# ywz978020607/MASIC

Measured on AMD Instinct MI355X. Metric: stereo pairs/sec (enc+dec), higher is better.
Workload: dtype bf16; 1 GPU; HSIC(N=128,M=192,K=5) eval forward (enc+dec both views), 8x3x512x512 stereo pairs per GPU (BASELINE.json configs[1] shape), inputs resident in HBM (the graph's static input buffers); the device homography of batch k+1 is handed over with batch k (one-batch look-ahead of a loader): its device->host read, the float32 host chain and the upload of the sampling matrices are done every step, under the r; pairs_per_gpu=8, height=512, width=512, parallelism=dp1 (pairs sharded, no data-path collective)

## Files before the change

coremasic/mywork/MASIC.py:

```python
import math
import os

import numpy as np

import torch
import torch.nn as nn
import torch.nn.functional as F

from compressai.entropy_models import (EntropyBottleneck, GaussianConditional, GaussianMixtureConditional,
                                       GaussianMixtureConditional_gf)
from compressai.layers import GDN, MaskedConv2d, ResidualBlock, conv3x3
from compressai.models.utils import conv, deconv, update_registered_buffers
from masic_amd import ops as _hip
from masic_amd.homography import warp_matrices as _warp_matrices
from masic_amd import autograd as _ag
from masic_amd.streams import ForkJoin as _ForkJoin
from masic_amd import fp8 as _fp8
from masic_amd import deconv as _deconv
from masic_amd import conv_s2 as _conv_s2
from masic_amd import latent as _latent
from masic_amd.bands import check_band_rows as _check_band_rows
from masic_amd.f16k import F16K as _F16K, F8K as _F8K

_RELU, _LEAKY, _NONE = _hip.ACT_RELU, _hip.ACT_LEAKY, _hip.ACT_NONE
_CAT_F16K = True
_HEADS_GROUPED = True


class CompressionModel(nn.Module):

    def __init__(self, entropy_bottleneck_channels, init_weights=True):
        super().__init__()
        self.entropy_bottleneck1 = EntropyBottleneck(entropy_bottleneck_channels)
        self.entropy_bottleneck2 = EntropyBottleneck(entropy_bottleneck_channels)
        if init_weights:
            self._initialize_weights()

    def aux_loss(self):
        return sum(m.loss() for m in self.modules() if isinstance(m, EntropyBottleneck))

    def _initialize_weights(self):
        for m in self.modules():
            if isinstance(m, (nn.Conv2d, nn.ConvTranspose2d)):
                nn.init.kaiming_normal_(m.weight)
                if m.bias is not None:
                    nn.init.zeros_(m.bias)

    def forward(self, *args):
        raise NotImplementedError()

    def parameters(self):
        for child in self.children():
            if not isinstance(child, EntropyBottleneck):
                yield from child.parameters()

    def aux_parameters(self):
        for child in self.children():
            if isinstance(child, EntropyBottleneck):
                yield from child.parameters()

    def update(self, force=False):
        for child in self.children():
            if isinstance(child, EntropyBottleneck):
                child.update(force=force)


class RateDistortionLoss(nn.Module):

    def __init__(self, lmbda=1e-2):
        super().__init__()
        self.lmbda = lmbda

    def forward(self, output, target):
        N, _, H, W = target.size()
        n = N * H * W
        bpp = sum(_hip.sum_log(l.contiguous()) for l in output["likelihoods"].values()) / (-math.log(2) * n)
        mse = _hip.sse(output["x_hat"].contiguous(), target.contiguous()) / target.numel()
        return {"bpp_loss": bpp.float(), "mse_loss": mse.float(), "loss": (self.lmbda * 255 ** 2 * mse + bpp).float()}


class AverageMeter:
    def __init__(self):
        self.val = self.avg = self.sum = self.count = 0

    def update(self, val, n=1):
        self.val = val
        self.sum += val * n
        self.count += n
        self.avg = self.sum / self.count


_SIDE_STREAMS = {}


def _side_streams(device, n=4):
    key = torch.device(device).index
    pool = _SIDE_STREAMS.get(key)
    if pool is None:
        pool, seen = [], set()
        for _ in range(64):
            s = torch.cuda.Stream(device=device)
            if s.cuda_stream not in seen:
                seen.add(s.cuda_stream)
                pool.append(s)
            if len(pool) == n + 1:
                break
        pool = _SIDE_STREAMS[key] = tuple(pool)
    cur = torch.cuda.current_stream(device).cuda_stream
    return tuple(s for s in pool if s.cuda_stream != cur)[:n]


_TRAIN_STREAMS = os.environ.get("MASIC_TRAIN_STREAMS", "1") != "0"


def _keep_until(t, stream):
    if not (torch.is_tensor(t) or isinstance(t, _F16K)):
        return
    if not torch.cuda.is_current_stream_capturing():
        t.record_stream(stream)


def _bf16_inference(*tensors):
    from masic_amd import nn as _mnn
    if not _mnn.reduced_precision():
        return False
    return not (torch.is_grad_enabled() and any(t.requires_grad for t in tensors))


def _f16k_chain(convs, acts, x, in_op=0, out=None, out_coff=0, gate=None, gate_c=0):
    B, _, H, W = x.shape
    hw = (H, W)
    for cv in convs:
        if not cv.f16k_supported(B, *hw):
            return None
        hw = cv.out_hw(*hw)
    t = x if isinstance(x, _F16K) else _F16K.from_nchw(x, in_op=in_op)
    for cv, act in zip(convs[:-1], acts):
        t = cv.run_f16k(t, act=act)
    return convs[-1].run_f16k(t, act=acts[-1], want_nchw=out is None, out=out, out_coff=out_coff, gate=gate, gate_c=gate_c)


def _pair_conv(conv, xa, xb, gdn_in=None, gdn_out=None):
    B, _, H, W = xa.shape
    desc = conv._desc((B, 6, H, W))
    def g(m):
        return None if m is None else (m.beta.detach(), m.gamma.detach().contiguous(), m.inverse)
    bm = (gdn_in or gdn_out).beta_min if (gdn_in or gdn_out) is not None else 1e-6
    return _hip.conv5s1_pair(xa, xb, conv.packed_weight(desc), None if conv.bias is None else conv.bias.detach(),
                             gdn_in=g(gdn_in), gdn_out=g(gdn_out), beta_min=bm)


def _gdn_f16k(gdn, x):
    return _hip.gdn_f16k(x, gdn.beta.detach(), gdn.gamma.detach(), inverse=gdn.inverse, beta_min=gdn.beta_min)


def _own_kernel_or_f16k(kernel, cv, gdn, t):
    if t.whole and kernel.supported(cv, gdn, t.B, t.H, t.W):
        return kernel.run(cv, gdn, t)
    return cv.run_f16k(t, gdn=gdn)


def _analysis_f16k(owner, x, layouts=None):
    from masic_amd import nn as _mnn
    convs = (owner.g_a_conv1, owner.g_a_conv2, owner.g_a_conv3, owner.g_a_conv4)
    gdns = (owner.g_a_gdn1, owner.g_a_gdn2, owner.g_a_gdn3)
    B, C, H, W = x.shape
    c1 = convs[0]
    if (C, c1.out_channels, tuple(c1.kernel_size), tuple(c1.stride), tuple(c1.padding)) != (3, 128, (5, 5), (2, 2), (2, 2)):
        return None
    sizes = [((H - 1) // 2 + 1, (W - 1) // 2 + 1)]
    for cv in convs[1:]:
        if not cv.f16k_supported(B, *sizes[-1]):
            return None
# ... 87 lines not shown
                L = dict(x=t[k], bias=layer.bias.detach(), Cin=layer.in_channels, Cout=layer.out_channels, act=acts[i],
                         out="nchw" if i == 2 else "f16k")
                if sc is not None and i < 2:
                    L["wp"], L["ws"] = layer.packed_gemm_f8k_weight(sc["c"] if i == 0 else sc[tag])
                    if i == 0:
                        L["out"], L["out_scale"] = "f8k", sc[tag]
                else:
                    L["wp"] = layer.packed_gemm_dma_weight()
                layers.append(L)
            t = _hip.gemm_f16k_group(layers, B, H, W)
        return tuple(t)

    def _f8k_heads_ok(self):
        return all(seq[i].in_channels % 32 == 0 and seq[i].out_channels % 32 == 0 for seq in (self.gmm_sigma, self.gmm_means, self.gmm_weights) for i in (0, 2)) \
            and all(seq[4].in_channels % 16 == 0 and seq[4].out_channels % 32 == 0 for seq in (self.gmm_sigma, self.gmm_means, self.gmm_weights))

    def heads(self, x, parallel=True):
        from masic_amd import nn as _mnn
        if isinstance(x, _F16K):
            if not x.whole:
                raise RuntimeError(f"_GmmHeads.heads: the grouped GEMMs read a whole buffer, not {x!r}")
            return self._heads_grouped(x, None)
        if _mnn.reduced_precision() and not (torch.is_grad_enabled() and (x.requires_grad or self.gmm_sigma[0].weight.requires_grad)):
            B, _, H, W = x.shape
            sc = _fp8.scales(self)
            use_f8 = sc is not None and self._f8k_heads_ok()
            if use_f8:
                xv = _F8K(_hip.nchw_to_f8k(x, sc["c"]), *x.shape, sc["c"])
                branch = lambda seq, tag, acts: self._branch_f8k(seq, xv, sc, tag, acts)
            else:
                xv = _F16K.from_nchw(x)
                xf = xv.buf

                def branch(seq, tag, acts):
                    if _fp8.recording():
                        _fp8.record(self, "c", x)
                        l0 = seq[0]
                        _fp8.record(self, tag, _hip.gemm_f16k(xf, l0.packed_gemm_dma_weight(), l0.bias.detach(), B, l0.in_channels, l0.out_channels, H, W, acts[0])
                                    if l0.in_channels % 16 == 0 and l0.out_channels % 32 == 0 else
                                    _hip.gemm1x1_bf16(xf, l0.packed_gemm_weight(), l0.bias.detach(), B, l0.in_channels, l0.out_channels, H, W, acts[0]))
                    return self._branch_f16k(seq, xv, acts)
            if _HEADS_GROUPED and not _fp8.recording() and self._grouped_heads_ok():
                return self._heads_grouped(xv, sc if use_f8 else None)
            if not parallel:
                return (branch(self.gmm_sigma, "h_sigma", (_RELU, _RELU, _RELU)),
                        branch(self.gmm_means, "h_means", (_LEAKY, _LEAKY, _NONE)),
                        branch(self.gmm_weights, "h_weights", (_LEAKY, _LEAKY, _NONE)))
            fj = _ForkJoin()
            cur = fj.main
            side = _side_streams(x.device)[2:4]
            outs = [None, None, None]
            for i, (st, (seq, tag, acts)) in enumerate(zip(side, ((self.gmm_means, "h_means", (_LEAKY, _LEAKY, _NONE)),
                                                                  (self.gmm_weights, "h_weights", (_LEAKY, _LEAKY, _NONE))))):
                fj.fork(st)
                with fj.on(st):
                    outs[i + 1] = branch(seq, tag, acts)
            outs[0] = branch(self.gmm_sigma, "h_sigma", (_RELU, _RELU, _RELU))
            for st in side:
                fj.join(st)
            for t in outs[1:] + [xv.buf]:
                _keep_until(t, cur)
            return tuple(outs)
        if torch.is_grad_enabled() and _ag.gmm_heads_supported(self, x):
            return _ag.gmm_heads(self, x)
        sigma = self._branch(self.gmm_sigma, x, (_RELU, _RELU, _RELU))
        means = self._branch(self.gmm_means, x, (_LEAKY, _LEAKY, _NONE))
        logits = self._branch(self.gmm_weights, x, (_LEAKY, _LEAKY, _NONE))
        return sigma, means, logits

    def forward(self, x):
        sigma, means, logits = self.heads(x)
        return sigma, means, _hip.softmax_k(logits, self.K)


class gmm_hyper_y1_same_resolution(_GmmHeads):

    def __init__(self, N, M, K):
        super().__init__()
        self.N, self.M, self.K = N, M, K
        self.gmm_sigma = nn.Sequential(
            deconv(4 * M, 6 * M, kernel_size=1, stride=1), nn.ReLU(inplace=True),
            deconv(6 * M, 4 * M, kernel_size=1, stride=1), nn.ReLU(inplace=True),
            conv(4 * M, M * K, kernel_size=1, stride=1), nn.ReLU(inplace=True))
        self.gmm_means = nn.Sequential(
            deconv(4 * M, 6 * M, kernel_size=1, stride=1), nn.LeakyReLU(inplace=True),
            deconv(6 * M, 4 * M, kernel_size=1, stride=1), nn.LeakyReLU(inplace=True),
            conv(4 * M, M * K, kernel_size=1, stride=1))
        self.gmm_weights = nn.Sequential(
            deconv(4 * M, 6 * M, kernel_size=1, stride=1), nn.LeakyReLU(inplace=True),
            deconv(6 * M, M * K, kernel_size=1, stride=1), nn.LeakyReLU(inplace=True),
            conv(M * K, M * K, kernel_size=1, stride=1))


class gmm_hyper_y2_same_resolution(_GmmHeads):

    def __init__(self, N, M, K):
        super().__init__()
        self.N, self.M, self.K = N, M, K
        self.gmm_sigma = nn.Sequential(
            conv(5 * M, 6 * M, kernel_size=1, stride=1), nn.ReLU(inplace=True),
            conv(6 * M, 4 * M, kernel_size=1, stride=1), nn.ReLU(inplace=True),
            conv(4 * M, M * K, kernel_size=1, stride=1), nn.ReLU(inplace=True))
        self.gmm_means = nn.Sequential(
            conv(5 * M, 6 * M, kernel_size=1, stride=1), nn.LeakyReLU(inplace=True),
            conv(6 * M, 4 * M, kernel_size=1, stride=1), nn.LeakyReLU(inplace=True),
            conv(4 * M, M * K, kernel_size=1, stride=1))
        self.gmm_weights = nn.Sequential(
            conv(5 * M, 6 * M, kernel_size=1, stride=1), nn.LeakyReLU(inplace=True),
            conv(6 * M, M * K, kernel_size=1, stride=1), nn.LeakyReLU(inplace=True),
            conv(M * K, M * K, kernel_size=1, stride=1))


class mask2weights(nn.Module):

    def __init__(self, N, M, Kw):
        super().__init__()
        self.maskconv = nn.Sequential(
            conv(1, 3, kernel_size=3, stride=2), nn.ReLU(inplace=True),
            conv(3, 6, kernel_size=3), nn.ReLU(inplace=True),
            conv(6, 6, kernel_size=3), nn.ReLU(inplace=True),
            conv(6, 3, kernel_size=3))
        self.N, self.M, self.Kw = N, M, Kw

    def forward(self, m):
        s = self.maskconv
        t = s[0].run(m, act=_RELU)
        t = s[2].run(t, act=_RELU)
        t = s[4].run(t, act=_RELU)
        return s[6].run(t, act=_hip.ACT_SOFTMAX_C)


def _synthesis_f16k(dec, y_hat):
    B, _, H, W = y_hat.shape
    convs = (dec.g_s_conv1, dec.g_s_conv2, dec.g_s_conv3)
    gdns = (dec.g_s_gdn1, dec.g_s_gdn2, dec.g_s_gdn3)
    sizes = [(H, W)]
    for cv in convs:
        if cv.out_channels != 128 or not cv.f16k_supported(B, *sizes[-1]):
            return None
        sizes.append(cv.out_hw(*sizes[-1]))
    if not dec.g_s_conv4.d2s_supported(B, *sizes[3]):
        return None
    t = y_hat if isinstance(y_hat, _F16K) else _F16K.from_nchw(y_hat)
    sc = _fp8.scales(dec)
    if sc is not None and convs[1].f8k_supported(B, *sizes[1]) and convs[2].f8k_supported(B, *sizes[2]):
        t = convs[0].run_f16k_f8out(t, sc["d1"], gdn=gdns[0])
        t = convs[1].run_f8k(t, gdn=gdns[1], out="f8k", out_scale=sc["d2"])
        t = convs[2].run_f8k(t, gdn=gdns[2], out="f16k")
        return dec.g_s_conv4.run_f16k_d2s(t)
    for i in range(3):
        t = _own_kernel_or_f16k(_deconv, convs[i], gdns[i], t)
        if i < 2:
            _fp8.record(dec, "d%d" % (i + 1), t.buf)
    return dec.g_s_conv4.run_f16k_d2s(t)


class Encoder1(nn.Module):

    def __init__(self, N, M, **kwargs):
        super().__init__()
        self.g_a_conv1 = conv(3, N)
        self.g_a_gdn1 = GDN(N)
        self.g_a_conv2 = conv(N, N)
        self.g_a_gdn2 = GDN(N)
        self.g_a_conv3 = conv(N, N)
        self.g_a_gdn3 = GDN(N)
        self.g_a_conv4 = conv(N, M)

    def forward(self, x):
        g1 = self.g_a_gdn1(self.g_a_conv1(x))
        g2 = self.g_a_gdn2(self.g_a_conv2(g1))
        g3 = self.g_a_gdn3(self.g_a_conv3(g2))
        return self.g_a_conv4(g3), g1, g2, g3

    def latent(self, x):
        if _bf16_inference(x, self.g_a_conv1.weight):
            y = _analysis_f16k(self, x.contiguous())
            if y is not None:
                return y
        return self.forward(x)[0]

    def latent_layouts(self, x, **layouts):
        if _bf16_inference(x, self.g_a_conv1.weight):
            return _analysis_f16k(self, x.contiguous(), layouts=layouts)
        return None

    def latent_train(self, x):
        if _ag.analysis_supported(self, x):
            return _ag.analysis(self, x)
        return self.forward(x)[0]


class Decoder1(nn.Module):

    def __init__(self, N, M, **kwargs):
        super().__init__()
        self.g_s_conv1 = deconv(M, N)
        self.g_s_gdn1 = GDN(N, inverse=True)
        self.g_s_conv2 = deconv(N, N)
        self.g_s_gdn2 = GDN(N, inverse=True)
        self.g_s_conv3 = deconv(N, N)
        self.g_s_gdn3 = GDN(N, inverse=True)
        self.g_s_conv4 = deconv(N, 3)

    def forward(self, y_hat):
        g1 = self.g_s_gdn1(self.g_s_conv1(y_hat))
        g2 = self.g_s_gdn2(self.g_s_conv2(g1))
        g3 = self.g_s_gdn3(self.g_s_conv3(g2))
        return self.g_s_conv4(g3), g1, g2, g3

    def reconstruct(self, y_hat):
        if isinstance(y_hat, _F16K):
            return _synthesis_f16k(self, y_hat) if _bf16_inference(self.g_s_conv1.weight) else None
        if _bf16_inference(y_hat, self.g_s_conv1.weight):
            x_hat = _synthesis_f16k(self, y_hat)
            if x_hat is not None:
                return x_hat
        return self.forward(y_hat)[0]

    def reconstruct_train(self, y_hat):
        if _ag.synthesis_supported(self, y_hat):
            return _ag.synthesis(self, y_hat)
        return self.forward(y_hat)[0]


class Encoder2(nn.Module):

    def __init__(self, N, M, **kwargs):
        super().__init__()
        self.pre_conv = conv(6, 3, stride=1)
        self.pre_gdn = GDN(3)
        self.g_a_conv1 = conv(3, N)
        self.g_a_gdn1 = GDN(N)
        self.g_a_conv2 = conv(N, N)
        self.g_a_gdn2 = GDN(N)
        self.g_a_conv3 = conv(N, N)
        self.g_a_gdn3 = GDN(N)
        self.g_a_conv4 = conv(N, M)

    def forward(self, x1_warp, x2):
        if not (torch.is_grad_enabled() and (x1_warp.requires_grad or x2.requires_grad or self.pre_conv.weight.requires_grad)):
            return self.forward_views(x1_warp, x2)
        return self.forward_pair(_ag.cat(x1_warp, x2))

    def forward_views(self, x1_warp, x2, layouts=None):
        t = _pair_conv(self.pre_conv, x1_warp.contiguous(), x2.contiguous(), gdn_out=self.pre_gdn)
        if layouts is not None and _bf16_inference(t, self.g_a_conv1.weight):
            lay = _analysis_f16k(self, t, layouts=layouts)
            if lay is not None:
                return lay
        return self._analysis(t)

    def forward_pair(self, pair):
        return self._analysis(self.pre_gdn(self.pre_conv(pair)))

    def _analysis(self, t):
        if _bf16_inference(t, self.g_a_conv1.weight):
            y = _analysis_f16k(self, t)
            if y is not None:
                return y
        if torch.is_grad_enabled() and _ag.analysis_supported(self, t):
            return _ag.analysis(self, t)
        t = self.g_a_gdn1(self.g_a_conv1(t))
        t = self.g_a_gdn2(self.g_a_conv2(t))
        t = self.g_a_gdn3(self.g_a_conv3(t))
        return self.g_a_conv4(t)


class Decoder2(nn.Module):

    def __init__(self, N, M, **kwargs):
        super().__init__()
        self.g_s_conv1 = deconv(M, N)
        self.g_s_gdn1 = GDN(N, inverse=True)
        self.g_s_conv2 = deconv(N, N)
        self.g_s_gdn2 = GDN(N, inverse=True)
        self.g_s_conv3 = deconv(N, N)
        self.g_s_gdn3 = GDN(N, inverse=True)
        self.g_s_conv4 = deconv(N, 3)
        self.after_gdn = GDN(3, inverse=True)
        self.after_conv = deconv(6, 3, stride=1)

    def forward(self, y_hat, x1_hat_warp):
        if isinstance(y_hat, _F16K):
            t = _synthesis_f16k(self, y_hat) if _bf16_inference(x1_hat_warp, self.g_s_conv1.weight) else None
            if t is None:
                return None
        else:
            t = _synthesis_f16k(self, y_hat) if _bf16_inference(y_hat, self.g_s_conv1.weight) else None
        if t is None and torch.is_grad_enabled() and _ag.synthesis_supported(self, y_hat):
            t = _ag.synthesis(self, y_hat)
        if t is None:
            t = self.g_s_gdn1(self.g_s_conv1(y_hat))
            t = self.g_s_gdn2(self.g_s_conv2(t))
            t = self.g_s_gdn3(self.g_s_conv3(t))
            t = self.g_s_conv4(t)
        if not (torch.is_grad_enabled() and (t.requires_grad or x1_hat_warp.requires_grad or self.after_conv.weight.requires_grad)):
            return _pair_conv(self.after_conv, t.contiguous(), x1_hat_warp.contiguous(), gdn_in=self.after_gdn)
        t = self.after_gdn(t)
        return self.after_conv(_ag.cat(t, x1_hat_warp))


def mask(im1, H_inv):
    B, _, h, w = im1.shape
    m_fwd, m_back = _warp_matrices(H_inv, (h, w), (h, w), want_inverse=True)
    mask_r = _hip.warp_perspective(None, m_fwd, (h, w), ones_like=(B, h, w))
# ... 967 lines not shown
```

masic_amd/nn.py:

```python
import torch
import torch.nn as nn

import os

from . import ops
from .f16k import F16K, F8K
from ._lib import PREC_BF16, PREC_F32, PREC_FP8

_PRECISION = {"f32": PREC_F32, "bf16": PREC_BF16, "fp8": PREC_BF16}[os.environ.get("MASIC_PRECISION", "f32")]
_FP8 = os.environ.get("MASIC_PRECISION", "f32") == "fp8"


def set_precision(name):
    global _PRECISION, _FP8
    _PRECISION = {"f32": PREC_F32, "bf16": PREC_BF16, "fp8": PREC_BF16}[name]
    _FP8 = name == "fp8"


def get_precision():
    return "fp8" if _FP8 else ("bf16" if _PRECISION == PREC_BF16 else "f32")


def reduced_precision():
    return _PRECISION == PREC_BF16
# ... 31 lines not shown
        for k, v in m.__dict__.items():
            if k.endswith("_cache") and isinstance(v, tuple):
                stack = list(v[1:])
                while stack:
                    x = stack.pop()
                    if isinstance(x, torch.Tensor):
                        out.append(x)
                    elif isinstance(x, dict):
                        stack.extend(x.values())
                    elif isinstance(x, (tuple, list)):
                        stack.extend(x)
    return out


def packed_gdn_f16k(gdn):
    key = weight_key(gdn.beta) + weight_key(gdn.gamma)
    cache = gdn.__dict__.get("_packed_f16k_cache")
    if cache is None or cache[0] != key:
        cache = (key, ops.pack_gdn_f16k(gdn.beta.detach(), gdn.gamma.detach().contiguous(), gdn.beta_min))
        gdn.__dict__["_packed_f16k_cache"] = cache
    return cache[1]


class _PackedWeightMixin:
    transposed_conv = False
    masked_conv = False

    def _geometry(self):
        kh, kw = _pair(self.kernel_size)
        sh, sw = _pair(self.stride)
        ph, pw = _pair(self.padding)
        if sh != sw or ph != pw or _pair(self.dilation) != (1, 1) or self.groups != 1:
            raise RuntimeError("masic_amd: only square stride/padding, dilation 1, groups 1 convolutions are built")
        if self.transposed_conv and _pair(self.output_padding) != (sh - 1, sh - 1):
            raise RuntimeError("masic_amd: ConvTranspose2d needs output_padding = stride - 1 (compressai deconv())")
        return kh, kw, sh, ph

    def _desc(self, x_shape, in_ctot=None, in_coff=0, out_ctot=None, out_coff=0, in_op=ops.INOP_NONE,
              act=ops.ACT_NONE, gate_ctot=0, gate_c=0):
        kh, kw, s, p = self._geometry()
        B, _, Hi, Wi = x_shape
        return ops.make_conv_desc(B, self.in_channels, Hi, Wi, self.out_channels, kh, kw, s, p,
                                  transposed=self.transposed_conv, masked=self.masked_conv,
                                  in_ctot=in_ctot, in_coff=in_coff, out_ctot=out_ctot, out_coff=out_coff,
                                  in_op=in_op, act=act, gate_ctot=gate_ctot, gate_c=gate_c, prec=_PRECISION)

    def packed_weight(self, desc):
        w = self.weight
        return _cached(self, "_packed_cache", weight_key(w), (desc.B, desc.Hi, desc.Wi, desc.prec),
                       lambda: ops.pack_conv_weight(w.detach().contiguous(), desc))

    def packed_gemm_weight(self):
        w = self.weight
        key = weight_key(w)
        cache = self.__dict__.get("_packed_gemm_cache")
        if cache is None or cache[0] != key:
            cache = (key, ops.pack_gemm1x1_weight(w.detach().contiguous(), self.in_channels, self.out_channels, self.transposed_conv))
            self.__dict__["_packed_gemm_cache"] = cache
        return cache[1]

    def out_hw(self, Hi, Wi):
        kh, kw, s, p = self._geometry()
        return ops.conv_out_hw(Hi, Wi, kh, kw, s, p, self.transposed_conv)

    def _desc_f16k(self, B, Hi, Wi, out_ctot=None, out_coff=0, act=ops.ACT_NONE, gate_ctot=0, gate_c=0, in_ctot=None, in_coff=0):
        kh, kw, s, p = self._geometry()
        cin16 = (self.in_channels + 15) // 16 * 16
        return ops.make_conv_desc(B, self.in_channels, Hi, Wi, self.out_channels, kh, kw, s, p,
                                  transposed=self.transposed_conv, masked=self.masked_conv,
                                  in_ctot=cin16 if in_ctot is None else in_ctot, in_coff=in_coff,
                                  out_ctot=out_ctot, out_coff=out_coff, act=act, gate_ctot=gate_ctot, gate_c=gate_c, prec=PREC_BF16)

    def _desc_of(self, x, out=None, out_coff=0, act=ops.ACT_NONE, gate=None, gate_c=0, blk=16, nchw=False):
        if x.C != self.in_channels:
            raise RuntimeError(f"masic_amd: a layer of {self.in_channels} input channels on {x!r}")
        if isinstance(out, F16K):
            out_ctot, out_coff = out.ctot, out.coff
            if (out.B, out.C, out.H, out.W) != (x.B, self.out_channels) + self.out_hw(x.H, x.W):
                raise RuntimeError(f"masic_amd: {out!r} is not the output of this layer on {x!r}")
        elif out is not None:
            out_ctot = out.shape[1]
        else:
            out_ctot = None if nchw else (self.out_channels + blk - 1) // blk * blk
        return self._desc_f16k(x.B, x.H, x.W, out_ctot=out_ctot, out_coff=out_coff, act=act, gate_ctot=0 if gate is None else gate.shape[1],
                               gate_c=gate_c if gate is not None else 0, in_ctot=x.ctot, in_coff=x.coff)

    def _f16k_out(self, buf, desc, out=None):
        return out if out is not None else F16K(buf, desc.B, self.out_channels, desc.Ho, desc.Wo, desc.out_ctot, 0)

    def f16k_supported(self, B, Hi, Wi):
        return ops.conv_f16k_supported(self._desc_f16k(B, Hi, Wi))

    def packed_f16k_weight(self, desc):
        w = self.weight
        return _cached(self, "_packed_f16k_cache", weight_key(w), (desc.B, desc.Hi, desc.Wi),
                       lambda: ops.pack_conv_f16k_weight(w.detach().contiguous(), desc, persistent=w.is_contiguous() and not self.masked_conv))

    def _bias(self):
        return None if self.bias is None else self.bias.detach()

    def _desc_f8k(self, B, Hi, Wi, out_ctot=None, out_coff=0, act=ops.ACT_NONE, gate_ctot=0, gate_c=0):
        kh, kw, s, p = self._geometry()
        cin32 = (self.in_channels + 31) // 32 * 32
        return ops.make_conv_desc(B, self.in_channels, Hi, Wi, self.out_channels, kh, kw, s, p,
                                  transposed=self.transposed_conv, masked=self.masked_conv, in_ctot=cin32,
                                  out_ctot=out_ctot, out_coff=out_coff, act=act, gate_ctot=gate_ctot, gate_c=gate_c, prec=PREC_FP8)

    def f8k_supported(self, B, Hi, Wi):
        return self.in_channels % 32 == 0 and ops.conv_f16k_supported(self._desc_f8k(B, Hi, Wi))

    def run_f8k(self, x, act=ops.ACT_NONE, out="f16k", out_scale=None, out_nchw=None, out_coff=0, gate=None, gate_c=0, gdn=None):
        B, Hi, Wi = x.B, x.H, x.W
        gct = 0 if gate is None else gate.shape[1]
        if out_nchw is not None:
            desc = self._desc_f8k(B, Hi, Wi, out_ctot=out_nchw.shape[1], out_coff=out_coff, act=act, gate_ctot=gct, gate_c=gate_c)
        elif out == "nchw":
            desc = self._desc_f8k(B, Hi, Wi, act=act)
        else:
            blk = 32 if out == "f8k" else 16
            desc = self._desc_f8k(B, Hi, Wi, out_ctot=(self.out_channels + blk - 1) // blk * blk, act=act)
        w = self.weight
        vkey = weight_key(w)
        wp, ws = _cached(self, "_packed_f8k_cache", vkey, (desc.B, desc.Hi, desc.Wi), lambda: ops.pack_conv_f8k_weight(w.detach().contiguous(), desc))
        wscale = _cached(self, "_wscale_f8k_cache", vkey, (desc.B, desc.Hi, desc.Wi, float(x.scale)), lambda: (ws * float(x.scale)).contiguous())
        y = ops.conv2d_f8k(x.buf, wp, wscale, self._bias(), desc, out=out, out_scale=out_scale, out_nchw=out_nchw,
                           gate=gate, gdn=None if gdn is None else (packed_gdn_f16k(gdn), gdn.inverse))
        if out_nchw is not None or out == "nchw":
            return y
        if out == "f8k":
            return F8K(y, B, self.out_channels, desc.Ho, desc.Wo, out_scale)
        return self._f16k_out(y, desc)

    def run_f16k_f8out(self, x, out_scale, act=ops.ACT_NONE, gdn=None):
        desc = self._desc_of(x, act=act, blk=32)
        y = ops.conv2d_f8k(x.buf, self.packed_f16k_weight(desc), None, self._bias(), desc, out="f8k",
                           out_scale=out_scale, gdn=None if gdn is None else (packed_gdn_f16k(gdn), gdn.inverse))
        return F8K(y, x.B, self.out_channels, desc.Ho, desc.Wo, out_scale)

    def packed_gemm_f8k_weight(self, in_scale):
        w = self.weight
        vkey = weight_key(w)
        wp, ws = _cached(self, "_packed_gemm_f8k_cache", vkey, (), lambda: ops.pack_gemm_f8k_weight(w.detach().contiguous(), self.in_channels, self.out_channels, self.transposed_conv))
        return wp, _cached(self, "_wscale_gemm_f8k_cache", vkey, (float(in_scale),), lambda: (ws * float(in_scale)).contiguous())

    def packed_first_layer_weight(self):
        w = self.weight
        key = weight_key(w)
        cache = self.__dict__.get("_packed_conv_a_cache")
        if cache is None or cache[0] != key:
            cache = (key, ops.pack_conv_a_weight(w.detach().contiguous()))
            self.__dict__["_packed_conv_a_cache"] = cache
        return cache[1]

    def run_f16k_d2s(self, x, out=None, out_coff=0):
        if not self.transposed_conv or self._geometry() != (5, 5, 2, 2):
            raise RuntimeError("masic_amd: run_f16k_d2s is for ConvTranspose2d(k=5, s=2, p=2)")
        if not x.whole or x.C != self.in_channels:
            raise RuntimeError(f"masic_amd: run_f16k_d2s takes a whole tensor of {self.in_channels} channels, not {x!r}")
        B, Hi, Wi = x.B, x.H, x.W
        desc = ops.make_conv_desc(B, self.in_channels, Hi, Wi, 32, 3, 3, 1, 1, prec=PREC_BF16)
        w = self.weight

        def build():
            wc, bc = ops.deconv_s2_as_conv_weight_dev(w.detach().contiguous(), self._bias())
            return ops.pack_conv_f16k_weight(wc, desc), bc
        wp, bc = _cached(self, "_packed_d2s_cache", weight_key(w) + (None if self.bias is None else weight_key(self.bias),),
                         (B, Hi, Wi), build)
        return ops.conv2d_f16k_d2s(x.buf, wp, bc, desc, self.out_channels, out=out, out_coff=out_coff)

    def d2s_supported(self, B, Hi, Wi):
        return (self.transposed_conv and self._geometry() == (5, 5, 2, 2) and self.out_channels <= 8 and self.in_channels % 32 == 0
                and ops.conv_f16k_supported(ops.make_conv_desc(B, self.in_channels, Hi, Wi, 32, 3, 3, 1, 1, prec=PREC_BF16)))

    def run_f16k(self, x, act=ops.ACT_NONE, want_nchw=False, out=None, out_coff=0, gate=None, gate_c=0, gdn=None):
        to16 = isinstance(out, F16K)
        nchw = want_nchw or (out is not None and not to16)
        desc = self._desc_of(x, out, out_coff, act, gate if out is not None else None, gate_c, nchw=nchw)
        y = ops.conv2d_f16k(x.buf, self.packed_f16k_weight(desc), self._bias(), desc, out_nchw=None if to16 else out, want_nchw=want_nchw, gate=gate,
                            gdn=None if gdn is None else (packed_gdn_f16k(gdn), gdn.inverse), out16=out.buf if to16 else None)
        return y if nchw else self._f16k_out(y, desc, out)

    def f16k_multi_supported(self, B, Hi, Wi):
        return ops.conv_f16k_multi_supported(self._desc_f16k(B, Hi, Wi))

    def run_f16k_multi(self, x, want, round16=None, gate=None, gate_c=0):
        desc = self._desc_of(x, nchw=True)
        r = (None, 0, 0) if round16 is None else (round16.buf, round16.ctot, round16.coff)
        if round16 is not None and round16.shape != (x.B, self.out_channels, desc.Ho, desc.Wo):
            raise RuntimeError(f"masic_amd: {round16!r} is not the output of this layer on {x!r}")
        lay = ops.conv2d_f16k_multi(x.buf, self.packed_f16k_weight(desc), self._bias(), desc, want=want, round16=r[0], round16_ctot=r[1],
                                    round16_coff=r[2], gate=gate, gate_c=gate_c)
        for k in ("round16", "abs16"):
            if k in lay:
                lay[k] = round16 if (k == "round16" and round16 is not None) else F16K.wrap(lay[k], x.B, self.out_channels, desc.Ho, desc.Wo)
        return lay

    def run_f16k_dual(self, x, gdn, products=None):
        desc = self._desc_of(x)
        pre, y = ops.conv2d_f16k_gdn_dual(x.buf, self.packed_f16k_weight(desc), self._bias(), desc,
                                          (packed_gdn_f16k(gdn), gdn.inverse), products=products)
        return self._f16k_out(pre, desc), self._f16k_out(y, desc)

    def run_f16k_res(self, x, act=ops.ACT_NONE, res1=None, res2=None, out=None, y_pre=None):
        side = [r for r in (res1, res2, y_pre) if r is not None]
        res_ctot = side[0].ctot if side else 0
        for r in side:
            if not r.whole or r.ctot != res_ctot:
                raise RuntimeError(f"masic_amd: residual / pre-activation operands are whole tensors of one width, not {r!r}")
        res1, res2, y_pre = (None if r is None else r.buf for r in (res1, res2, y_pre))
        B, Hi, Wi = x.B, x.H, x.W
        if self.resident_supported(B, Hi, Wi) and act in (ops.ACT_NONE, ops.ACT_RELU, ops.ACT_LEAKY):
            w = self.weight
            wp = _cached(self, "_packed_c3_cache", weight_key(w), (), lambda: ops.pack_conv3x3_resident_weight(w.detach()))
            oc, ocoff = ((self.out_channels + 15) // 16 * 16, 0) if out is None else (out.ctot, out.coff)
            if not x.whole or (out is not None and out.shape != (B, self.out_channels, Hi, Wi)):
                raise RuntimeError(f"masic_amd: the resident-weight kernel takes a whole input and writes its own output, not {x!r} -> {out!r}")
            y = ops.conv3x3_resident(x.buf, wp, self._bias(), B, self.in_channels, self.out_channels, Hi, Wi, act=act, y16=None if out is None else out.buf,
                                     out_ctot=oc, out_coff=ocoff, res1=res1, res2=res2, res_ctot=res_ctot, y_pre=y_pre)
            return out if out is not None else F16K(y, B, self.out_channels, Hi, Wi, oc, 0)
        desc = self._desc_of(x, out, act=act)
        y = ops.conv2d_f16k_res(x.buf, self.packed_f16k_weight(desc), self._bias(), desc, y16=None if out is None else out.buf,
                                res1=res1, res2=res2, res_ctot=res_ctot, y_pre=y_pre)
        return self._f16k_out(y, desc, out)

    def resident_supported(self, B, Hi, Wi):
        return (not self.transposed_conv and not self.masked_conv and self._geometry() == (3, 3, 1, 1)
                and ops.conv3x3_resident_supported(B, self.in_channels, self.out_channels, Hi, Wi))

    def few_supported(self, B, Hi, Wi):
        kh, kw, s_, p_ = self._geometry()
        return (not self.transposed_conv and self.out_channels <= 32 and self.in_channels % 16 == 0
                and ops.conv_f16k_supported(ops.make_conv_desc(B, self.in_channels, Hi, Wi, 32, kh, kw, s_, p_, prec=PREC_BF16)))

    def run_f16k_few(self, x, res32=None):
        if not x.whole or x.C != self.in_channels:
            raise RuntimeError(f"masic_amd: run_f16k_few takes a whole tensor of {self.in_channels} channels, not {x!r}")
        B, Hi, Wi = x.B, x.H, x.W
        kh, kw, s_, p_ = self._geometry()
        desc = ops.make_conv_desc(B, self.in_channels, Hi, Wi, 32, kh, kw, s_, p_, prec=PREC_BF16)
        w = self.weight
        vkey = weight_key(w) + (None if self.bias is None else weight_key(self.bias),)

        def build():
            wpad = torch.zeros((32,) + tuple(w.shape[1:]), dtype=torch.float32, device=w.device)
            wpad[:self.out_channels] = w.detach()
            bpad = torch.zeros(32, dtype=torch.float32, device=w.device)
            if self.bias is not None:
                bpad[:self.out_channels] = self.bias.detach()
            return ops.pack_conv_f16k_weight(wpad, desc), bpad
        wp, bp = _cached(self, "_packed_few_cache", vkey, (B, Hi, Wi), build)
        return ops.conv2d_f16k_few(x.buf, wp, bp, desc, self.out_channels, res32=res32)

    def packed_gemm_dma_weight(self):
        w = self.weight
        key = weight_key(w)
        cache = self.__dict__.get("_packed_gemm_dma_cache")
        if cache is None or cache[0] != key:
            cache = (key, ops.pack_gemm_f16k_weight(w.detach().contiguous(), self.in_channels, self.out_channels, self.transposed_conv))
            self.__dict__["_packed_gemm_dma_cache"] = cache
        return cache[1]

    def run(self, x, in_coff=0, out=None, out_coff=0, in_op=ops.INOP_NONE, act=ops.ACT_NONE, gate=None, gate_c=0,
            res1=None, res2=None):
        if torch.is_grad_enabled() and (x.requires_grad or self.weight.requires_grad):
            return self._run_autograd(x, in_coff, out, in_op, act, gate, gate_c, res1, res2)
        desc = self._desc(x.shape, in_ctot=x.shape[1], in_coff=in_coff,
                          out_ctot=None if out is None else out.shape[1], out_coff=out_coff,
                          in_op=in_op, act=act, gate_ctot=0 if gate is None else gate.shape[1], gate_c=gate_c)
        bias = None if self.bias is None else self.bias.detach()
        return ops.conv2d(x, self.packed_weight(desc), bias, desc, out=out, gate=gate, res1=res1, res2=res2)

    def f16k_out_supported(self, shape):
        return reduced_precision() and ops.conv2d_f16k_out_supported(self._desc(tuple(shape), out_ctot=(self.out_channels + 15) // 16 * 16))

    def run_f16k_out(self, x, act=ops.ACT_NONE):
        desc = self._desc(tuple(x.shape), out_ctot=(self.out_channels + 15) // 16 * 16, act=act)
        return self._f16k_out(ops.conv2d_f16k_out(x, self.packed_weight(desc), self._bias(), desc), desc)

    def _run_autograd(self, x, in_coff, out, in_op, act, gate, gate_c, res1, res2):
        from . import autograd as A
        if out is not None:
            raise RuntimeError("masic_amd: writing into a concat buffer is an inference-only fusion; use autograd.CatFn when training")
        if in_coff != 0 or x.shape[1] != self.in_channels:
            raise RuntimeError("masic_amd: channel-slice inputs are an inference-only fusion")
        if in_op == ops.INOP_ABS:
            x = A.AbsFn.apply(x)
        elif in_op != ops.INOP_NONE:
            raise RuntimeError("masic_amd: round() inputs have no gradient path (eval-mode fusion)")
        if act == ops.ACT_SOFTMAX_C:
            y = A.SoftmaxKFn.apply(A.conv(self, x), self.out_channels)
        else:
            y = A.conv(self, x, act)
        if gate is not None:
            y = A.GateFn.apply(y, gate, gate_c)
        for r in (res1, res2):
            if r is not None:
                y = A.AddFn.apply(y, r)
        return y

    def forward(self, x):
        return self.run(x)


class Conv2d(_PackedWeightMixin, nn.Conv2d):
    pass


class ConvTranspose2d(_PackedWeightMixin, nn.ConvTranspose2d):
    transposed_conv = True

    def forward(self, x, output_size=None):
        if output_size is not None:
            raise RuntimeError("masic_amd: ConvTranspose2d(output_size=...) is not supported")
        return self.run(x)
```

Measured before the change: 4568 stereo pairs/s.

## Add warp-specialized persistent kernel for final depth-to-space deconv layer

Adds a dedicated HIP kernel for the last 128->C 5x5 stride-2 transposed conv, computed as a 3x3 conv followed by depth-to-space. Four loader waves stream the weights and input patches into a four-deep LDS ring with buffer DMA, while eight compute waves run bf16 MFMA and write NCHW float output directly. Tiles are grouped per XCD by image. The decoder uses this kernel only on the non-fp8 path, and only when a tile-count heuristic and a kernel-name check against the existing row kernel both pass. This adds a large hand-scheduled kernel with inline waitcnt and barrier logic, which carries correctness and maintenance risk.

```diff
diff --git a/coremasic/mywork/MASIC.py b/coremasic/mywork/MASIC.py
--- a/coremasic/mywork/MASIC.py
+++ b/coremasic/mywork/MASIC.py
@@ -19,6 +19,7 @@
 from masic_amd import deconv as _deconv
 from masic_amd import conv_s2 as _conv_s2
 from masic_amd import latent as _latent
+from masic_amd import d2s_layer as _d2s_layer
 from masic_amd.bands import check_band_rows as _check_band_rows
 from masic_amd.f16k import F16K as _F16K, F8K as _F8K
 
@@ -412,6 +413,8 @@
         t = _own_kernel_or_f16k(_deconv, convs[i], gdns[i], t)
         if i < 2:
             _fp8.record(dec, "d%d" % (i + 1), t.buf)
+    if t.whole and _d2s_layer.supported(dec.g_s_conv4, t.B, t.H, t.W) and _d2s_layer.preferred(dec.g_s_conv4, t.B, t.H, t.W):
+        return _d2s_layer.run(dec.g_s_conv4, t)
     return dec.g_s_conv4.run_f16k_d2s(t)
 
 
diff --git a/include/masic_d2s.h b/include/masic_d2s.h
--- /dev/null
+++ b/include/masic_d2s.h
@@ -0,0 +1,23 @@
+#ifndef MASIC_D2S_H
+#define MASIC_D2S_H
+
+#include <stddef.h>
+
+#ifdef __cplusplus
+extern "C" {
+#endif
+
+int masic_d2s_layer_f16k_supported(int B, int Hi, int Wi);
+
+int masic_d2s_layer_f16k_preferred(int B, int Hi, int Wi);
+
+int masic_d2s_layer_f16k_fwd(const void* x_f16k, const void* w_packed, const float* bias, float* y_nchw, int C, int y_ctot, int y_coff,
+                             int B, int Hi, int Wi, int max_wgs, void* stream);
+
+int masic_d2s_layer_f16k_kernel_name(int B, int Hi, int Wi, char* buf, size_t n);
+
+#ifdef __cplusplus
+}
+#endif
+
+#endif
diff --git a/masic_amd/csrc/d2s_layer.hip b/masic_amd/csrc/d2s_layer.hip
--- /dev/null
+++ b/masic_amd/csrc/d2s_layer.hip
@@ -0,0 +1,249 @@
+#include "f16k_device.h"
+#include "f16k_layer.h"
+#include "masic_d2s.h"
+
+namespace {
+
+struct D2sArgs {
+    const unsigned short* x;
+    const unsigned char* w;
+    const float* bias;
+    float* y;
+    int C, y_ctot, y_coff;
+    int Hi, Wi, tiles_w, tpi, ntiles, xcd_images;
+};
+
+constexpr int DL_CIN = 128, DL_CHUNKS = DL_CIN / 16;
+constexpr int DL_TAPS = 9, DL_STREAM_TAPS = 10;
+constexpr int DL_STREAM = DL_CHUNKS * DL_STREAM_TAPS * 4096;
+constexpr int DL_WBYTES = DL_CHUNKS * DL_TAPS * 1024;
+constexpr int DL_TH = 16, DL_TW = 32;
+constexpr int DL_PH = DL_TH + 2, DL_PW = DL_TW + 2, DL_NPIX = DL_PH * DL_PW;
+constexpr int DL_NI = (2 * DL_NPIX + 63) / 64;
+constexpr int DL_PB = DL_NI * 1024;
+constexpr int DL_NBUF = 4, DL_PD = DL_NBUF - 1;
+constexpr int DL_NLW = 4;
+constexpr int DL_NIW = DL_NI / DL_NLW, DL_NWW = DL_WBYTES / 1024 / DL_NLW;
+constexpr int DL_PATCH0 = DL_WBYTES, DL_LDS = DL_PATCH0 + DL_NBUF * DL_PB;
+constexpr int DL_MAX_WGS = 256;
+static_assert(DL_NIW * DL_NLW == DL_NI && DL_NWW * DL_NLW * 1024 == DL_WBYTES, "every loader wave moves the same number of pieces");
+static_assert(DL_NWW + DL_PD * DL_NIW <= 60 && DL_LDS <= 160 * 1024, "vmcnt is 6 bits; LDS");
+
+__device__ __forceinline__ void dl_barrier() {
+    asm volatile("" ::: "memory");
+    __builtin_amdgcn_s_barrier();
+    asm volatile("" ::: "memory");
+}
+
+__global__ __launch_bounds__(768, 1) void d2s_layer_f16k(const D2sArgs a) {
+    extern __shared__ __attribute__((aligned(1024))) unsigned char lds[];
+    const unsigned ldsb = (unsigned)(size_t)(__attribute__((address_space(3))) unsigned char*)lds;
+
+    const int tid = threadIdx.x, lane = tid & 63;
+    const int wave = __builtin_amdgcn_readfirstlane(tid >> 6);
+    const int j = lane & 31, h = lane >> 5;
+
+    const int xcd = a.xcd_images ? (int)(blockIdx.x & 7) : 0;
+    const int first = a.xcd_images ? (int)(blockIdx.x >> 3) : (int)blockIdx.x;
+    const int stride = a.xcd_images ? (int)(gridDim.x >> 3) : (int)gridDim.x;
+    const int n_my = first < a.ntiles ? (a.ntiles - first + stride - 1) / stride : 0;
+    if (n_my == 0) return;
+    const int plane_bytes = a.Hi * a.Wi * 32;
+    auto tile_of = [&](int i, int& b, int& r0, int& c0) {
+        const int idx = first + i * stride;
+        const int img = idx / a.tpi, rem = idx - img * a.tpi;
+        const int th_i = rem / a.tiles_w;
+        b = a.xcd_images ? img * 8 + xcd : img;
+        r0 = th_i * DL_TH;
+        c0 = (rem - th_i * a.tiles_w) * DL_TW;
+    };
+    const int ngroups = n_my * DL_CHUNKS;
+
+    if (wave >= 8) {
+        const int lw = wave - 8;
+        int prc[DL_NIW];
+#pragma unroll
+        for (int k = 0; k < DL_NIW; ++k) {
+            const int q = (k * DL_NLW + lw) * 64 + lane;
+            const int hh = q >= DL_NPIX ? 1 : 0, pp = q - hh * DL_NPIX;
+            const int pr = pp / DL_PW, pc = pp - pr * DL_PW;
+            prc[k] = q < 2 * DL_NPIX ? (hh << 16 | pr << 8 | pc) : -1;
+        }
+        const __amdgpu_buffer_rsrc_t rw = layer_rsrc(a.w, DL_STREAM);
+#pragma unroll
+        for (int k = 0; k < DL_NWW; ++k) {
+            const int piece = k * DL_NLW + lw;
+            const int c = piece / DL_TAPS, t = piece - c * DL_TAPS;
+            dma_buf16(rw, lds + piece * 1024, j * 16 + h * 2048, (c * DL_STREAM_TAPS + t) * 4096);
+        }
+        int goff[DL_NIW];
+        const unsigned short* xb = a.x;
+        auto issue = [&](int g) {
+            const int i = g >> 3, c = g & 7;
+            if (c == 0) {
+                int b = 0, r0 = 0, c0 = 0;
+                if (i < n_my) {
+                    tile_of(i, b, r0, c0);
+                    xb = a.x + (size_t)b * DL_CHUNKS * (size_t)(a.Hi * a.Wi * 16);
+                }
+#pragma unroll
+                for (int k = 0; k < DL_NIW; ++k) {
+                    const int ih = r0 - 1 + ((prc[k] >> 8) & 0xff), iw = c0 - 1 + (prc[k] & 0xff);
+                    const bool ok = i < n_my && prc[k] >= 0 && ih >= 0 && ih < a.Hi && iw >= 0 && iw < a.Wi;
+                    goff[k] = ok ? (ih * a.Wi + iw) * 32 + (prc[k] >> 16) * 16 : LAYER_OOB;
+                }
+            }
+            const __amdgpu_buffer_rsrc_t rx = layer_rsrc(xb, DL_CHUNKS * plane_bytes);
+            unsigned char* dst = lds + DL_PATCH0 + (g & (DL_NBUF - 1)) * DL_PB;
+#pragma unroll
+            for (int k = 0; k < DL_NIW; ++k) dma_buf16(rx, dst + (k * DL_NLW + lw) * 1024, goff[k], c * plane_bytes);
+        };
+#pragma unroll
+        for (int g = 0; g < DL_PD; ++g) issue(g);
+        asm volatile("s_waitcnt vmcnt(%0)" ::"n"((DL_PD - 1) * DL_NIW) : "memory");
+        dl_barrier();
+        for (int g = 0; g < ngroups; ++g) {
+            issue(g + DL_PD);
+            asm volatile("s_waitcnt vmcnt(%0)" ::"n"((DL_PD - 1) * DL_NIW) : "memory");
+            dl_barrier();
+        }
+        asm volatile("s_waitcnt vmcnt(0)" ::: "memory");
+        return;
+    }
+
+    float bv[16];
+#pragma unroll
+    for (int e = 0; e < 16; ++e) bv[e] = a.bias != nullptr ? a.bias[4 * h + (e & 3) + 8 * (e >> 2)] : 0.0f;
+    const unsigned wa = ldsb + lane * 16;
+    const unsigned pbl = ldsb + DL_PATCH0 + (h * DL_NPIX + 2 * wave * DL_PW + j) * 16;
+    const size_t oplane = (size_t)a.Hi * a.Wi;
+    dl_barrier();
+    for (int i = 0; i < n_my; ++i) {
+        f32x16 acc[2];
+#pragma unroll
+        for (int n = 0; n < 2; ++n)
+#pragma unroll
+            for (int e = 0; e < 16; ++e) acc[n][e] = bv[e];
+        for (int c = 0; c < DL_CHUNKS; ++c) {
+            const unsigned pb = pbl + ((i * DL_CHUNKS + c) & (DL_NBUF - 1)) * DL_PB, wc = wa + c * (DL_TAPS * 1024);
+            v4u bf[4][3], af[DL_TAPS];
+            auto read_b = [&](auto rc) {
+                constexpr int rr = decltype(rc)::value;
+                ds_read128<(rr * DL_PW + 0) * 16>(bf[rr][0], pb);
+                ds_read128<(rr * DL_PW + 1) * 16>(bf[rr][1], pb);
+                ds_read128<(rr * DL_PW + 2) * 16>(bf[rr][2], pb);
+            };
+            auto read_a = [&](auto uc) {
+                constexpr int u = decltype(uc)::value;
+                ds_read128<(3 * u + 0) * 1024>(af[3 * u + 0], wc);
+                ds_read128<(3 * u + 1) * 1024>(af[3 * u + 1], wc);
+                ds_read128<(3 * u + 2) * 1024>(af[3 * u + 2], wc);
+            };
+            auto taps = [&](auto uc) {
+                constexpr int u = decltype(uc)::value;
+                static_for<0, 2>([&](auto nc) {
+                    constexpr int n = decltype(nc)::value;
+                    static_for<0, 3>([&](auto vc) {
+                        constexpr int v = decltype(vc)::value;
+                        acc[n] = __builtin_amdgcn_mfma_f32_32x32x16_bf16(__builtin_bit_cast(bf16x8, af[3 * u + v]), __builtin_bit_cast(bf16x8, bf[n + u][v]), acc[n], 0, 0, 0);
+                    });
+                });
+            };
+            read_b(std::integral_constant<int, 0>{});
+            read_b(std::integral_constant<int, 1>{});
+            read_a(std::integral_constant<int, 0>{});
+            read_b(std::integral_constant<int, 2>{});
+            read_a(std::integral_constant<int, 1>{});
+            lgkm_wait<6>(bf[0][0], bf[0][1], bf[0][2], bf[1][0], bf[1][1], bf[1][2]);
+            lgkm_wait<6>(af[0], af[1], af[2]);
+            taps(std::integral_constant<int, 0>{});
+            __builtin_amdgcn_sched_barrier(0);
+            read_b(std::integral_constant<int, 3>{});
+            read_a(std::integral_constant<int, 2>{});
+            lgkm_wait<6>(bf[2][0], bf[2][1], bf[2][2], af[3], af[4], af[5]);
+            taps(std::integral_constant<int, 1>{});
+            lgkm_wait<0>(bf[3][0], bf[3][1], bf[3][2], af[6], af[7], af[8]);
+            taps(std::integral_constant<int, 2>{});
+            const v4u zero = {0u, 0u, 0u, 0u};
+            acc[0] = __builtin_amdgcn_mfma_f32_32x32x16_bf16(__builtin_bit_cast(bf16x8, zero), __builtin_bit_cast(bf16x8, bf[0][0]), acc[0], 0, 0, 0);
+            acc[1] = __builtin_amdgcn_mfma_f32_32x32x16_bf16(__builtin_bit_cast(bf16x8, zero), __builtin_bit_cast(bf16x8, bf[1][0]), acc[1], 0, 0, 0);
+            dl_barrier();
+        }
+        int b, r0, c0;
+        tile_of(i, b, r0, c0);
+#pragma unroll
+        for (int n = 0; n < 2; ++n) {
+            const int r = r0 + 2 * wave + n, cx = c0 + j;
+            if (r < a.Hi && cx < a.Wi) {
+                float* yb = a.y + ((size_t)b * a.y_ctot + a.y_coff) * (4 * oplane) + (size_t)(2 * r) * (2 * a.Wi) + 2 * cx;
+#pragma unroll
+                for (int q = 0; q < 4; ++q) {
+                    const int cc = h + 2 * q;
+                    if (cc < a.C) {
+                        float* yc = yb + (size_t)cc * (4 * oplane);
+                        *reinterpret_cast<float2*>(yc) = make_float2(acc[n][4 * q], acc[n][4 * q + 1]);
+                        *reinterpret_cast<float2*>(yc + 2 * a.Wi) = make_float2(acc[n][4 * q + 2], acc[n][4 * q + 3]);
+                    }
+                }
+            }
+        }
+    }
+}
+
+struct D2sPlan {
+    int tiles_w, tpi, ntiles, xcd_images, grid;
+};
+
+constexpr long long DL_ROW_MIN_TILES = 512;
+constexpr long long DL_PREFERRED_MIN_TILES = 512;
+
+long long d2s_row_tiles(int B, int Hi, int Wi) { return Wi >= 32 ? (long long)ceil_div(Wi, 32) * ceil_div(Hi, 32) * B : 0; }
+
+bool d2s_shape_ok(int B, int Hi, int Wi) {
+    return layer_shape_ok(B, Hi, Wi, 256) && (long long)ceil_div(Wi, DL_TW) * ceil_div(Hi, DL_TH) * B < (1ll << 27);
+}
+
+D2sPlan d2s_plan(int B, int Hi, int Wi, int max_wgs) {
+    D2sPlan p{};
+    p.tiles_w = ceil_div(Wi, DL_TW);
+    p.tpi = p.tiles_w * ceil_div(Hi, DL_TH);
+    const int cap = max_wgs > 0 && max_wgs < DL_MAX_WGS ? max_wgs : DL_MAX_WGS;
+    p.xcd_images = B % 8 == 0 && cap >= 8;
+    if (p.xcd_images) {
+        p.ntiles = B / 8 * p.tpi;
+        p.grid = 8 * (cap / 8 < p.ntiles ? cap / 8 : p.ntiles);
+    } else {
+        p.ntiles = B * p.tpi;
+        p.grid = cap < p.ntiles ? cap : p.ntiles;
+    }
+    return p;
+}
+
+}
+
+extern "C" int masic_d2s_layer_f16k_supported(int B, int Hi, int Wi) { return d2s_shape_ok(B, Hi, Wi) ? 1 : 0; }
+
+extern "C" int masic_d2s_layer_f16k_preferred(int B, int Hi, int Wi) {
+    if (!d2s_shape_ok(B, Hi, Wi)) return 0;
+    const long long t = d2s_row_tiles(B, Hi, Wi);
+    return t >= DL_ROW_MIN_TILES && t >= DL_PREFERRED_MIN_TILES ? 1 : 0;
+}
+
+extern "C" int masic_d2s_layer_f16k_kernel_name(int B, int Hi, int Wi, char* buf, size_t n) {
+    MASIC_REQUIRE(buf && n > 0 && d2s_shape_ok(B, Hi, Wi), MASIC_ERR_ARG, "d2s_layer_f16k_kernel_name: bad arguments");
+    MASIC_REQUIRE((size_t)snprintf(buf, n, "d2s_layer_f16k") < n, MASIC_ERR_ARG, "d2s_layer_f16k_kernel_name: buffer of %zu bytes too small", n);
+    return MASIC_OK;
+}
+
+extern "C" int masic_d2s_layer_f16k_fwd(const void* x_f16k, const void* w_packed, const float* bias, float* y_nchw, int C, int y_ctot, int y_coff,
+                                        int B, int Hi, int Wi, int max_wgs, void* stream) {
+    MASIC_REQUIRE(x_f16k && w_packed && y_nchw, MASIC_ERR_ARG, "d2s_layer_f16k_fwd: null pointer");
+    MASIC_REQUIRE(d2s_shape_ok(B, Hi, Wi), MASIC_ERR_UNSUPPORTED, "d2s_layer_f16k_fwd: %d x %d x %d is not supported", B, Hi, Wi);
+    MASIC_REQUIRE(C > 0 && 4 * C <= 32 && max_wgs >= 0, MASIC_ERR_UNSUPPORTED, "d2s_layer_f16k_fwd: needs 0 < C <= 8 and max_wgs >= 0");
+    MASIC_REQUIRE(y_coff >= 0 && y_coff + C <= y_ctot, MASIC_ERR_SHAPE, "d2s_layer_f16k_fwd: output channel view out of range");
+    const D2sPlan p = d2s_plan(B, Hi, Wi, max_wgs);
+    const D2sArgs a{(const unsigned short*)x_f16k, (const unsigned char*)w_packed, bias, y_nchw, C, y_ctot, y_coff,
+                    Hi, Wi, p.tiles_w, p.tpi, p.ntiles, p.xcd_images};
+    launch_lds<d2s_layer_f16k>(dim3(p.grid), 768, DL_LDS, (hipStream_t)stream, a);
+    return masic_launch_status("d2s_layer_f16k_fwd");
+}
diff --git a/masic_amd/d2s_layer.py b/masic_amd/d2s_layer.py
--- /dev/null
+++ b/masic_amd/d2s_layer.py
@@ -0,0 +1,89 @@
+import ctypes
+import functools
+import os
+
+import torch
+
+from . import _lib, ops
+from .f16k import F16K
+from .ops import _p, _stream
+
+IN_CHANNELS, MAX_OUT_CHANNELS = 128, 8
+PACKED_BYTES = 8 * 5 * 2 * 4096
+ROW = "conv_f16k<1, 2, 3, 5, 2, false, 1, 4, false>"
+
+HEADER_PATH = os.path.join(os.path.dirname(_lib.HEADER_PATH), "masic_d2s.h")
+SIGNATURES = _lib.bind_header(HEADER_PATH, "masic_d2s_")
+_WHO = "masic_amd.d2s_layer"
+
+
+def conv_desc(B, Hi, Wi):
+    return ops.make_conv_desc(B, IN_CHANNELS, Hi, Wi, 32, 3, 3, 1, 1, prec=_lib.PREC_BF16)
+
+
+@functools.lru_cache(maxsize=256)
+def takes_row(B, Hi, Wi):
+    buf = ctypes.create_string_buffer(96)
+    rc = _lib.lib.masic_conv_f16k_kernel_name(ctypes.byref(conv_desc(B, Hi, Wi)), _lib.F16K_NOSPLIT, buf, 96)
+    return rc == 0 and buf.value.decode() == ROW
+
+
+def kernel_name(B, Hi, Wi):
+    buf = ctypes.create_string_buffer(96)
+    _lib.check(_lib.lib.masic_d2s_layer_f16k_kernel_name(B, Hi, Wi, buf, 96), "d2s_layer_f16k_kernel_name")
+    return buf.value.decode()
+
+
+def launch(x16, packed, bias, B, Hi, Wi, C, out=None, out_coff=0, max_wgs=0):
+    if x16.dtype != torch.int16 or not x16.is_cuda or x16.numel() != B * IN_CHANNELS * Hi * Wi:
+        raise RuntimeError(f"{_WHO}: input must be an F16K int16 CUDA buffer of [{B},{IN_CHANNELS},{Hi},{Wi}]")
+    if packed.dtype != torch.int16 or packed.numel() * 2 != PACKED_BYTES or packed.device != x16.device:
+        raise RuntimeError(f"{_WHO}: `packed` is not the slab stream of the 128 -> 32 3x3 layer")
+    if bias is not None:
+        ops._dev(bias, "bias")
+        if bias.numel() != 32 or bias.device != x16.device:
+            raise RuntimeError(f"{_WHO}: bias must hold 32 values on the input's device")
+    if not 0 < C <= MAX_OUT_CHANNELS:
+        raise RuntimeError(f"{_WHO}: 1 to {MAX_OUT_CHANNELS} output channels, not {C}")
+    if not _lib.lib.masic_d2s_layer_f16k_supported(B, Hi, Wi):
+        raise RuntimeError(f"{_WHO}: shape [{B},{IN_CHANNELS},{Hi},{Wi}] is not supported")
+    if out is None:
+        out_coff = 0
+        out = torch.empty((B, C, 2 * Hi, 2 * Wi), dtype=torch.float32, device=x16.device)
+    else:
+        ops._dev(out, "output")
+        if (out.dim() != 4 or (out.shape[0], out.shape[2], out.shape[3]) != (B, 2 * Hi, 2 * Wi) or out.device != x16.device
+                or not 0 <= out_coff <= out.shape[1] - C):
+            raise RuntimeError(f"{_WHO}: `out` is not a float32 [{B}, >= {out_coff + C}, {2 * Hi}, {2 * Wi}] tensor on the input's device")
+    timed = None
+    if ops._timer is not None:
+        timed = ops._timer_open(conv_desc(B, Hi, Wi), lambda d, buf, n: _lib.lib.masic_d2s_layer_f16k_kernel_name(B, Hi, Wi, buf, n))
+    _lib.check(_lib.lib.masic_d2s_layer_f16k_fwd(_p(x16), _p(packed), _p(bias), _p(out), C, out.shape[1], out_coff, B, Hi, Wi, max_wgs,
+                                                 _stream()), "d2s_layer_f16k_fwd")
+    if timed is not None:
+        ops._timer_close(timed)
+    return out
+
+
+def supported(cv, B, Hi, Wi, in_ctot=None, in_coff=0, prec=_lib.PREC_BF16):
+    if not getattr(cv, "transposed_conv", False) or getattr(cv, "masked_conv", True):
+        return False
+    if cv.in_channels != IN_CHANNELS or not 0 < cv.out_channels <= MAX_OUT_CHANNELS or cv._geometry() != (5, 5, 2, 2):
+        return False
+    if prec != _lib.PREC_BF16 or in_coff != 0 or in_ctot not in (None, IN_CHANNELS):
+        return False
+    if not _lib.lib.masic_d2s_layer_f16k_supported(B, Hi, Wi) or not cv.d2s_supported(B, Hi, Wi):
+        return False
+    return takes_row(B, Hi, Wi)
+
+
+def preferred(cv, B, Hi, Wi):
+    return bool(_lib.lib.masic_d2s_layer_f16k_preferred(B, Hi, Wi))
+
+
+def run(cv, x, out=None, out_coff=0):
+    if not isinstance(x, F16K) or not x.whole or x.C != IN_CHANNELS or not supported(cv, x.B, x.H, x.W):
+        raise RuntimeError(f"{_WHO}: run takes whole 128-channel tensors and the 128 -> C <= 8 5x5 stride-2 transposed layer at the shapes of "
+                           f"{ROW}, not {x!r} on {cv!r}")
+    _, wp, bc = cv.packed_d2s(x.B, x.H, x.W)
+    return launch(x.buf, wp, bc, x.B, x.H, x.W, cv.out_channels, out=out, out_coff=out_coff)
diff --git a/masic_amd/nn.py b/masic_amd/nn.py
--- a/masic_amd/nn.py
+++ b/masic_amd/nn.py
@@ -207,20 +207,23 @@
             self.__dict__["_packed_conv_a_cache"] = cache
         return cache[1]
 
+    def packed_d2s(self, B, Hi, Wi):
+        desc = ops.make_conv_desc(B, self.in_channels, Hi, Wi, 32, 3, 3, 1, 1, prec=PREC_BF16)
+        w = self.weight
+
+        def build():
+            wc, bc = ops.deconv_s2_as_conv_weight_dev(w.detach().contiguous(), self._bias())
+            return ops.pack_conv_f16k_weight(wc, desc), bc
+        wp, bc = _cached(self, "_packed_d2s_cache", weight_key(w) + (None if self.bias is None else weight_key(self.bias),),
+                         (B, Hi, Wi), build)
+        return desc, wp, bc
+
     def run_f16k_d2s(self, x, out=None, out_coff=0):
         if not self.transposed_conv or self._geometry() != (5, 5, 2, 2):
             raise RuntimeError("masic_amd: run_f16k_d2s is for ConvTranspose2d(k=5, s=2, p=2)")
         if not x.whole or x.C != self.in_channels:
             raise RuntimeError(f"masic_amd: run_f16k_d2s takes a whole tensor of {self.in_channels} channels, not {x!r}")
-        B, Hi, Wi = x.B, x.H, x.W
-        desc = ops.make_conv_desc(B, self.in_channels, Hi, Wi, 32, 3, 3, 1, 1, prec=PREC_BF16)
-        w = self.weight
-
-        def build():
-            wc, bc = ops.deconv_s2_as_conv_weight_dev(w.detach().contiguous(), self._bias())
-            return ops.pack_conv_f16k_weight(wc, desc), bc
-        wp, bc = _cached(self, "_packed_d2s_cache", weight_key(w) + (None if self.bias is None else weight_key(self.bias),),
-                         (B, Hi, Wi), build)
+        desc, wp, bc = self.packed_d2s(x.B, x.H, x.W)
         return ops.conv2d_f16k_d2s(x.buf, wp, bc, desc, self.out_channels, out=out, out_coff=out_coff)
 
     def d2s_supported(self, B, Hi, Wi):
```

Result: faster. 4634 stereo pairs/s, median of 6 (+1.4%).
